# linyicheng1/trackingBench-SLAM

Measured on AMD Instinct MI355X. Metric: frames/sec end-to-end (extract+match+local-BA), higher is better.
Workload: dtype u8 (pyramid/FAST/ORB/Hamming) + f64 (pose-opt/BA); 1 GPU; 1280x720 stereo, 8-level pyramid x0.8, 2000 kpts/image (FAST 80/30), searchByBF L<->R, pose-opt, 10-KF/5000-pt local BA x10 iters; distinct_synthetic_pairs=64, distinct_ba_windows=32, ba_partitions=3, ba_schedule=joined at the end of every step, parallelism=frames sharded x1, RCCL gather of tracks

## Files before the change

### trackingbench_slam_amd/csrc/k_ba.hip

```cpp
#include <mutex>
#include <type_traits>
#include "tb_internal.h"
#include "tb_device.h"
#include "tb_se3.h"

#define BA_T 256
#ifndef BA_KFCH
#define BA_KFCH 512
#endif
#ifndef BA_KFBLK
#define BA_KFBLK 4
#endif
#define BA_BIG_MAXF 64
#define BA_SMALL_MAXF 10
#define BA_SORT_LDS 8192
#ifndef BA_EMAX
#define BA_EMAX 64
#endif
#ifndef BA_PCAP
#define BA_PCAP 21
#endif

struct BaState {
    double lambda, ni, currentChi, chi0, scale_p, rho;
    int iter, qmax, status, need_lin, cur, ok2, done_iters, err;
    int sing, pad0, hq_fresh, pad2;
};

struct BaDims {
    int W, nkf, nfixed, nfree, np, npt, obs_pitch, iters;
    int nblkP, kfChunks, G, nChunks;
    int Gbase, Gextra;
    int Vbase, Vextra;
    int big, npairs;
    unsigned long long oBigA;
    unsigned long long oPairStart, oPairCnt, oPairItems, maxItems;
    double fx, fy, cx, cy;
    unsigned long long wstride, oT, oP, oHll, oBl, oHq, oHpp, oBp, oXp, oPartKF, oPartP, oPartS;
    unsigned long long istride, oPtStart, oPtFree, oKfStart, oKfEdges, oFreeKP;
    unsigned long long oKfRec;
    unsigned long long oPtMask, oPermA, oPermB, oPtRank, oKPs, oGDesc;
    unsigned long long oGCost;
    unsigned long long oGCut;
    int renum;
    unsigned long long oPerm;
    int schurWaveLds;
    int wgReduce;
};

__host__ __device__ inline int ba_schur_waves(const BaDims& d, int w) {
    return d.wgReduce ? 4 * (d.Gbase + (w < d.Gextra ? 1 : 0)) : d.Vbase + (w < d.Vextra ? 1 : 0);
}
__device__ __forceinline__ void ba_schur_unit(int u, int base, int extra, int& w, int& i) {
// ... 2 lines not shown
    else { const int r = u - head; w = extra + r / base; i = r - (w - extra) * base; }
}

typedef double ba_d4 __attribute__((ext_vector_type(4)));
typedef double ba_d2 __attribute__((ext_vector_type(2)));

__device__ __forceinline__ double ba_huber_rho0(double c, double delta) {
    const double dsqr = delta * delta;
    return (c <= dsqr) ? c : 2 * sqrt(c) * delta - dsqr;
}
struct BaLin { double ww, e0, e1, c2, invz; double pc[3]; double Jl[6]; };
__device__ __forceinline__ double ba_rcp(double x) {
    double r = __builtin_amdgcn_rcp(x);
    r = fma(fma(-x, r, 1.0), r, r);
    r = fma(fma(-x, r, 1.0), r, r);
    return r;
}
__device__ __forceinline__ void ba_residual(const double* Rt, const double* X, float u, float v, float inv_sigma2, double fx,
                                            double fy, double cx, double cy, double delta, BaLin& L) {
#pragma unroll
    for (int i = 0; i < 3; i++) L.pc[i] = fma(Rt[3 * i + 2], X[2], fma(Rt[3 * i + 1], X[1], fma(Rt[3 * i], X[0], Rt[9 + i])));
    L.invz = ba_rcp(L.pc[2]);
    L.e0 = (double)u - fma(L.pc[0] * L.invz, fx, cx);
    L.e1 = (double)v - fma(L.pc[1] * L.invz, fy, cy);
    const double wgt = (double)inv_sigma2;
    L.c2 = fma(L.e0, wgt * L.e0, L.e1 * (wgt * L.e1));
    const double r1 = (L.c2 <= delta * delta) ? 1.0 : delta / sqrt(L.c2);
    L.ww = r1 * wgt;
}
__device__ __forceinline__ void ba_linearize(const double* Rt, const double* X, float u, float v, float inv_sigma2, double fx,
// ... 151 lines not shown
            [&](int e, int ce, bool hit) {
                const int prev = (e > 0) ? obs[e - 1].pt : -1, cur = obs[e].pt;
                for (int p = max(prev + 1, 0); p <= min(cur, d.npt); p++) I[d.oPtFree + p] = ce;
                if (hit) {
                    const tb_ba_obs o = obs[e];
                    int4 r;
                    r.x = (int)(((unsigned)cur << 6) | ((unsigned)(o.kf - d.nfixed) & 63u));
                    r.y = __float_as_int(o.u); r.z = __float_as_int(o.v); r.w = __float_as_int(o.inv_sigma2);
                    *reinterpret_cast<int4*>(I + d.oFreeKP + 4 * (size_t)ce) = r;
                }
            });
        for (int p = max((nobs > 0 ? obs[nobs - 1].pt : -1) + 1, 0) + tid; p <= d.npt; p += BA_T) I[d.oPtFree + p] = nfreeE;
        return;
    }
    if (tid == 0) {
        st->lambda = 0; st->ni = 2; st->currentChi = 0; st->chi0 = 0; st->scale_p = 0; st->rho = 0;
        st->iter = 0; st->qmax = 0; st->status = (d.iters > 0 && nobs > 0) ? 0 : 1; st->need_lin = 1; st->cur = 0; st->ok2 = 1;
        st->done_iters = 0; st->err = 0; st->sing = 0; st->hq_fresh = 0;
    }
    __syncthreads();
    if (!d.renum) {
        for (int e = tid; e < nobs; e += BA_T) {
            const int prev = (e > 0) ? obs[e - 1].pt : -1, cur = obs[e].pt;
            for (int p = max(prev + 1, 0); p <= min(cur, d.npt); p++) I[d.oPtStart + p] = e;
        }
        for (int p = max((nobs > 0 ? obs[nobs - 1].pt : -1) + 1, 0) + tid; p <= d.npt; p += BA_T) I[d.oPtStart + p] = nobs;
        if (d.big) for (int p = tid; p < d.npt; p += BA_T) I[d.oPtRank + p] = p;
    }
    for (int kk = tid; kk < d.nkf; kk += BA_T) {
        const float* T = poses + ((size_t)w * d.nkf + kk) * 16;
        double R[9], t[3];
        for (int i = 0; i < 3; i++) { for (int j = 0; j < 3; j++) R[i * 3 + j] = (double)T[i * 4 + j]; t[i] = (double)T[i * 4 + 3]; }
        const PoSE3 s = po_from_Rt(R, t);
        ba_store_se3(D + d.oT + (size_t)kk * 7, s);
        ba_store_se3(D + d.oT + (size_t)(d.nkf + kk) * 7, s);
    }
    for (int i = tid; i < d.npt * 3; i += BA_T) {
        const int r = i / 3, c = i - 3 * r;
        const double v = (double)pts[(size_t)w * d.npt * 3 + (d.renum ? 3 * (size_t)I[d.oPerm + r] + c : (size_t)i)];
        D[d.oP + i] = v;
        D[d.oP + (size_t)d.npt * 3 + i] = v;
    }
}

__device__ __forceinline__ void ba_write_rec(double* q, const double* Hll, const double* bl, const double* X, double lambda,
                                             BaState* st) {
    const double a00 = Hll[0] + lambda, a10 = Hll[1], a20 = Hll[2], a11 = Hll[3] + lambda, a21 = Hll[4], a22 = Hll[5] + lambda;
    bool ok = a00 > 0;
    const double i00 = 1.0 / sqrt(ok ? a00 : 1.0), c10 = a10 * i00, c20 = a20 * i00;
    const double d1 = a11 - c10 * c10;
    ok = ok && d1 > 0;
    const double i11 = 1.0 / sqrt(ok ? d1 : 1.0), c21 = (a21 - c20 * c10) * i11;
    const double d2 = a22 - c20 * c20 - c21 * c21;
    ok = ok && d2 > 0 && isfinite(d2);
    const double i22 = 1.0 / sqrt(ok ? d2 : 1.0);
    if (!ok) st->sing = 1;
    const double u00 = i00, u11 = i11, u22 = i22, u01 = -c10 * i00 * i11, u12 = -c21 * i11 * i22,
                 u02 = -(c20 * i00 + c21 * u01) * i22;
    q[0] = ok ? u00 : 0.0; q[1] = ok ? u01 : 0.0; q[2] = ok ? u02 : 0.0;
    q[3] = ok ? u11 : 0.0; q[4] = ok ? u12 : 0.0; q[5] = ok ? u22 : 0.0;
    q[6] = bl[0]; q[7] = bl[1]; q[8] = bl[2];
    q[9] = X[0]; q[10] = X[1]; q[11] = X[2];
}
__device__ __forceinline__ void ba_rec_utb(const double* q, double* t) {
    t[0] = q[0] * q[6];
    t[1] = q[1] * q[6] + q[3] * q[7];
    t[2] = q[2] * q[6] + q[4] * q[7] + q[5] * q[8];
}

__device__ __forceinline__ void ba_points_pass(const BaDims& d, const tb_ba_obs* __restrict__ obsAll, double* __restrict__ dw, const int* __restrict__ iw,
                                               BaState* __restrict__ states, const int* __restrict__ errflag, int bx, int w) {
    __shared__ double red[4];
    extern __shared__ __attribute__((aligned(16))) double sRt[];
    const int tid = threadIdx.x;
    if (errflag[w]) {
        if (bx == 0 && tid == 0) { states[w].status = 1; states[w].err = 1; }
        return;
    }
    const BaState st = states[w];
    if (st.status) return;
    double* D = dw + (size_t)w * d.wstride;
    const int* I = iw + (size_t)w * d.istride;
    const bool lam_known = st.iter > 0 || !st.need_lin;
    const tb_ba_obs* obs = obsAll + (size_t)w * d.obs_pitch;
    const double* T = D + d.oT + (size_t)st.cur * d.nkf * 7;
    const double* P = D + d.oP + (size_t)st.cur * d.npt * 3;
    for (int k = tid; k < d.nkf; k += BA_T) ba_pose_to_Rt(T + k * 7, sRt + k * 12);
    __syncthreads();
    const double delta = (double)sqrtf(5.991f);
    const int p = bx * BA_T + tid;
    double chi = 0, maxd = 0;
    if (p < d.npt) {
        double Hll[6] = {0, 0, 0, 0, 0, 0}, bl[3] = {0, 0, 0};
        const double X[3] = {P[3 * p], P[3 * p + 1], P[3 * p + 2]};
        const int eBeg = I[d.oPtStart + p], eEnd = I[d.oPtStart + p + 1];
        tb_ba_obs on = obs[min(eBeg, d.obs_pitch - 1)];
        for (int e = eBeg; e < eEnd; e++) {
            const tb_ba_obs o = on;
            on = obs[min(e + 1, d.obs_pitch - 1)];
            BaLin L;
            ba_linearize(sRt + o.kf * 12, X, o.u, o.v, o.inv_sigma2, d.fx, d.fy, d.cx, d.cy, delta, L);
            const double ww = L.ww, e0 = L.e0, e1 = L.e1;
            const double* Jl = L.Jl;
            chi += ba_huber_rho0(L.c2, delta);
            for (int a = 0; a < 3; a++) bl[a] = fma(-ww, fma(Jl[a], e0, Jl[3 + a] * e1), bl[a]);
            Hll[0] = fma(ww, fma(Jl[0], Jl[0], Jl[3] * Jl[3]), Hll[0]);
            Hll[1] = fma(ww, fma(Jl[0], Jl[1], Jl[3] * Jl[4]), Hll[1]);
            Hll[2] = fma(ww, fma(Jl[0], Jl[2], Jl[3] * Jl[5]), Hll[2]);
            Hll[3] = fma(ww, fma(Jl[1], Jl[1], Jl[4] * Jl[4]), Hll[3]);
            Hll[4] = fma(ww, fma(Jl[1], Jl[2], Jl[4] * Jl[5]), Hll[4]);
            Hll[5] = fma(ww, fma(Jl[2], Jl[2], Jl[5] * Jl[5]), Hll[5]);
        }
        if (!lam_known) {
            for (int a = 0; a < 6; a++) D[d.oHll + (size_t)p * 6 + a] = Hll[a];
            for (int a = 0; a < 3; a++) D[d.oBl + (size_t)p * 3 + a] = bl[a];
        } else ba_write_rec(D + d.oHq + (size_t)I[d.oPtRank + p] * 12, Hll, bl, X, st.lambda, states + w);
        maxd = fmax(fabs(Hll[0]), fmax(fabs(Hll[3]), fabs(Hll[5])));
    }
    const double s = ba_block_sum1(chi, red);
    const double m = ba_block_max1(maxd, red);
    if (tid == 0) {
        D[d.oPartP + (size_t)bx * 4] = s;
        D[d.oPartP + (size_t)bx * 4 + 1] = m;
    }
}

#define BA_KFG 14
#define BA_KFR_LDS (4 * (BA_KFG * 65 + 64) + 4 * 27)
__device__ __forceinline__ double ba_block_sum27(const double (&v)[27], double* sh) {
    const int tid = threadIdx.x, wave = tid >> 6, lane = tid & 63;
    double* T = sh + wave * (BA_KFG * 65 + 64);
// ... 75 lines not shown
            for (int a = 0; a < 6; a++) {
                const double wa = ww * Jp[a], wb = ww * Jp[6 + a];
                acc[21 + a] -= fma(wa, e0, wb * e1);
#pragma unroll
                for (int c = a; c < 6; c++) {
                    const int at = a * 6 - (a * (a - 1)) / 2 + (c - a);
                    acc[at] += fma(wa, Jp[c], wb * Jp[6 + c]);
                }
            }
        }
        const double tot = ba_block_sum27(acc, red);
        if (tid < 27) D[d.oPartKF + ((size_t)kfree * d.kfChunks + chunk) * 27 + tid] = tot;
    }
}

__global__ void __launch_bounds__(BA_T)
k_ba_points(BaDims d, const tb_ba_obs* __restrict__ obsAll, double* __restrict__ dw, const int* __restrict__ iw, BaState* __restrict__ states,
            const int* __restrict__ errflag) {
    ba_points_pass(d, obsAll, dw, iw, states, errflag, (int)blockIdx.x, (int)blockIdx.y);
}
__global__ void __launch_bounds__(BA_T)
k_ba_kf(BaDims d, const tb_ba_obs* __restrict__ obsAll, double* __restrict__ dw, const int* __restrict__ iw, const BaState* __restrict__ states,
        const int* __restrict__ errflag) {
    ba_kf_pass(d, obsAll, dw, iw, states, errflag, (int)blockIdx.x);
}
__global__ void __launch_bounds__(BA_T)
k_ba_lin(BaDims d, const tb_ba_obs* __restrict__ obsAll, double* __restrict__ dw, const int* __restrict__ iw, BaState* __restrict__ states,
         const int* __restrict__ errflag, int nKfBlocks) {
    if ((int)blockIdx.x < nKfBlocks) ba_kf_pass(d, obsAll, dw, iw, states, errflag, (int)blockIdx.x);
    else {
        const int b = (int)blockIdx.x - nKfBlocks;
        ba_points_pass(d, obsAll, dw, iw, states, errflag, b % d.nblkP, b / d.nblkP);
    }
}

__device__ __forceinline__ void ba_reduce_body(const BaDims& d, double* __restrict__ dw, const int* __restrict__ iw, BaState* __restrict__ states,
                                               int w, double* red) {
    const int tid = threadIdx.x;
    BaState* st = states + w;
    double* D = dw + (size_t)w * d.wstride;
    const int* I = iw + (size_t)w * d.istride;
    double maxd = 0;
    for (int i = tid; i < d.nfree * 27; i += BA_T) {
        const int kf = i / 27, c = i - kf * 27;
        const int nedges = I[d.oKfStart + d.nfixed + kf + 1] - I[d.oKfStart + d.nfixed + kf];
        const int nch = (nedges + BA_KFCH - 1) / BA_KFCH;
        double s = 0;
        for (int ch = 0; ch < nch; ch++) s += D[d.oPartKF + ((size_t)kf * d.kfChunks + ch) * 27 + c];
        if (c >= 21) D[d.oBp + kf * 6 + (c - 21)] = s;
        else {
            int a = 0, rem = c;
            while (rem >= 6 - a) { rem -= 6 - a; a++; }
            const int b = a + rem;
            D[d.oHpp + (size_t)kf * 36 + a * 6 + b] = s;
            D[d.oHpp + (size_t)kf * 36 + b * 6 + a] = s;
            if (a == b) maxd = fmax(maxd, fabs(s));
        }
    }
    const double mH = ba_block_max1(maxd, red);
    if (tid == 0) {
        double chi = 0, mL = 0;
        for (int b = 0; b < d.nblkP; b++) { chi += D[d.oPartP + (size_t)b * 4]; mL = fmax(mL, D[d.oPartP + (size_t)b * 4 + 1]); }
        st->currentChi = chi;
        if (st->iter == 0) { st->chi0 = chi; st->lambda = 1e-5 * fmax(mH, mL); st->ni = 2; }
        st->hq_fresh = st->iter > 0 ? 1 : 0;
        st->need_lin = 0;
    }
}

__global__ void __launch_bounds__(BA_T)
k_ba_reduce(BaDims d, double* __restrict__ dw, const int* __restrict__ iw, BaState* __restrict__ states) {
    __shared__ double red[4];
    const int w = blockIdx.x;
    if (states[w].status || !states[w].need_lin) return;
    ba_reduce_body(d, dw, iw, states, w, red);
}

__global__ void __launch_bounds__(BA_T)
k_ba_hinv(BaDims d, double* __restrict__ dw, const int* __restrict__ iw, BaState* __restrict__ states) {
    const int w = blockIdx.y, p = blockIdx.x * BA_T + threadIdx.x;
    const BaState st = states[w];
    if (st.status || st.hq_fresh || p >= d.npt) return;
    double* D = dw + (size_t)w * d.wstride;
    const int* I = iw + (size_t)w * d.istride;
    double ph[6], pb[3], X[3];
#pragma unroll
    for (int i = 0; i < 6; i++) ph[i] = D[d.oHll + (size_t)p * 6 + i];
#pragma unroll
    for (int i = 0; i < 3; i++) { pb[i] = D[d.oBl + (size_t)p * 3 + i]; X[i] = D[d.oP + ((size_t)st.cur * d.npt + p) * 3 + i]; }
    ba_write_rec(D + d.oHq + (size_t)I[d.oPtRank + p] * 12, ph, pb, X, st.lambda, states + w);
}

#define BA_MAXT 4
#define BA_REC 12
#define BA_RECS_LDS 256
#define BA_KMFMA 5
#define BA_ZERO_LDS 40
__device__ __forceinline__ void ba_wave_lds_fence() { __builtin_amdgcn_fence(__ATOMIC_SEQ_CST, "wavefront"); }

__host__ __device__ constexpr int ba_c_cap(int k) { return (BA_EMAX / k) < BA_PCAP ? (BA_EMAX / k) : BA_PCAP; }
__host__ __device__ constexpr int ba_c_nb(int k) { return (6 * k + 1 + 3) / 4; }
__host__ __device__ constexpr int ba_c_ld(int k) { return ((3 * ba_c_cap(k) + 3) / 4) * 4 + 2; }
__host__ __device__ constexpr int ba_c_tile(int k) { return 4 * ba_c_nb(k) * ba_c_ld(k); }
#define BA_CB 37
__host__ __device__ constexpr int ba_c_rhs(int k) { return BA_CB * (k * (k + 1) / 2); }
__host__ __device__ constexpr int ba_c_tri(int k) { return ba_c_rhs(k) + 6 * k; }
__host__ __device__ constexpr int ba_c_nacc(int k) {
    const int nb = ba_c_nb(k), nvf = nb / 4, rem = nb % 4;
    return 3 * nvf + 2 * nvf * (nvf - 1) + rem * (nvf + 1);
// ... 613 lines not shown
    const int zeroOfs = d.schurWaveLds - BA_ZERO_LDS;
    double* D = dw + (size_t)w * d.wstride;
    const int* I = iw + (size_t)w * d.istride;
    for (int k = lane; k < d.nfree; k += 64) ba_pose_to_Rt(D + d.oT + ((size_t)st.cur * d.nkf + d.nfixed + k) * 7, sRtf + k * 12);
    double S[36];
#pragma unroll
    for (int e = 0; e < 36; e++) S[e] = 0;
    double rhs = 0;
    int pa = 0;
    while ((pa + 1) * (pa + 2) / 2 <= lane) pa++;
    const int pb = lane - pa * (pa + 1) / 2;
    if (lane < BA_ZERO_LDS) Zt[zeroOfs + lane] = 0;
    ba_wave_lds_fence();
    const double delta = (double)sqrtf(5.991f);
    const int lastE = d.obs_pitch - 1;
    const double* Hq = D + d.oHq;
    const int4* KPs = reinterpret_cast<const int4*>(I + d.oKPs);
    const int4* GD = reinterpret_cast<const int4*>(I + d.oGDesc);
    const unsigned lastQ = (unsigned)d.npt * BA_REC - 1u;
    const int gBeg = I[d.oGCut + wv], gEnd = I[d.oGCut + wv + 1], lastG = gEnd - 1;
    auto range = [&](BaPreC& X, int g) {
        X.nxt = GD[min(g, max(lastG, 0))];
        if (g > lastG) X.nxt.w = 0;
    };
    auto preload = [&](BaPreC& X, int g) {
        const int4 gd = X.nxt;
        const int4 r = KPs[(unsigned)min(gd.y + lane, lastE)];
        X.key = (lane < gd.w * __popc(gd.z)) ? r.x : -1;
        X.u = __int_as_float(r.y); X.v = __int_as_float(r.z); X.w = __int_as_float(r.w);
        const unsigned qb = (unsigned)gd.x * BA_REC + (unsigned)lane;
        X.r0 = Hq[min(qb, lastQ)];
// ... 41 lines not shown
        BA_TK(5);
        const int mask = __builtin_amdgcn_readfirstlane(X.cur.z), npts = __builtin_amdgcn_readfirstlane(X.cur.w);
        const int k = __popc(mask), ld = ba_ctab.ld[k];
        if (pend != 0 && pend != mask) { finish(pend); pend = 0; }
        BA_TK(3);
        Hi[lane] = X.r0;
        Hi[64 + lane] = X.r1;
        Hi[128 + lane] = X.r2;
        Hi[192 + lane] = X.r3;
        ba_wave_lds_fence();
        const bool live = X.key >= 0;
        const int pl = live ? (lane * ((65536 + k - 1) / k)) >> 16 : 0;
        const int slot = live ? lane - pl * k : 0, kf = live ? (X.key & 63) : 0;
        if (live) {
            const double* q = Hi + pl * BA_REC;
            const double u00 = q[0], u01 = q[1], u02 = q[2], u11 = q[3], u12 = q[4], u22 = q[5];
            const double Xp[3] = {q[9], q[10], q[11]};
            BaLin L;
            double Jp[12];
            ba_linearize(sRtf + kf * 12, Xp, X.u, X.v, X.w, d.fx, d.fy, d.cx, d.cy, delta, L);
            ba_jac_pose_iz(L.pc, L.invz, d.fx, d.fy, Jp);
            double JU[6];
#pragma unroll
            for (int r = 0; r < 2; r++) {
                JU[3 * r] = L.Jl[3 * r] * u00;
                JU[3 * r + 1] = fma(L.Jl[3 * r], u01, L.Jl[3 * r + 1] * u11);
                JU[3 * r + 2] = fma(L.Jl[3 * r], u02, fma(L.Jl[3 * r + 1], u12, L.Jl[3 * r + 2] * u22));
            }
            double* z = Zt + (6 * slot) * ld + 3 * pl;
#pragma unroll
            for (int i = 0; i < 6; i++) JU[i] *= L.ww;
#pragma unroll
            for (int a = 0; a < 6; a++) {
#pragma unroll
                for (int c = 0; c < 3; c++)
                    z[a * ld + c] = (a == 3) ? Jp[3] * JU[c] : (a == 4) ? Jp[10] * JU[3 + c] : fma(Jp[a], JU[c], Jp[6 + a] * JU[3 + c]);
            }
            if (slot == 0) {
                double* zr = Zt + (6 * k) * ld + 3 * pl;
                ba_rec_utb(q, zr);
            }
        }
        const int ncol = 3 * npts, nks = (ncol + 3) >> 2;
        if (lane <= 6 * k) {
#pragma unroll
            for (int c = 0; c < 3; c++)
                if (ncol + c < 4 * nks) Zt[lane * ld + ncol + c] = 0;
        }
        ba_wave_lds_fence();
        BA_TK(0);
        preload(X, g + 2);
        BA_TK(1);
        if (k <= BA_KMFMA) {
            switch (k) {
                case 1: ba_c_mac<1>(acc, Zt, nks, lane); break;
// ... 79 lines not shown
        }
    } else {
        double* out = D + d.oPartS + (size_t)wv * 64 * 64;
        if (lane < NPAIR) {
#pragma unroll
            for (int e = 0; e < 36; e++) out[(6 * pa + e / 6) * 64 + 6 * pb + e % 6] = S[e];
        }
        if (lane < d.np) out[lane * 64 + d.np] = rhs;
    }
#ifdef BA_TIMING
    BA_TK(9);
    if (tid == 0 && (w & 15) == 0) { for (int i = 0; i < 10; i++) atomicAdd(&ba_times[i], tk_[i]); atomicAdd(&ba_times[10], 1ull); }
#endif
}

__device__ __forceinline__ double ba_rsqrt(double x) {
    double r = __builtin_amdgcn_rsq(x);
    const double h = 0.5 * x;
    r = fma(r, fma(-h * r, r, 0.5), r);
    r = fma(r, fma(-h * r, r, 0.5), r);
    return r;
}
#define BA_SOLVE_T 256
template <int NS>
__global__ void __launch_bounds__(BA_SOLVE_T)
k_ba_solve(BaDims d, double* __restrict__ dw, const int* __restrict__ iw, BaState* __restrict__ states, int with_reduce) {
    __shared__ double A[64 * 65];
    __shared__ double x[64];
    __shared__ double Lcol[2][64];
    const int w = blockIdx.x, tid = threadIdx.x;
#ifdef BA_TIMING
    unsigned long long ts_[6]; ts_[0] = __builtin_readcyclecounter();
#endif
    BaState* st = states + w;
    if (with_reduce) {
        __shared__ double redf[4];
        if (st->status) return;
// ... 495 lines not shown
    }
    __syncthreads();
    const double* T = D + d.oT + (size_t)st->cur * d.nkf * 7;
    double* Tn = D + d.oT + (size_t)(st->cur ^ 1) * d.nkf * 7;
    for (int k = tid; k < d.nkf; k += BA_ST) {
        const PoSE3 Tk = ba_load_se3(T + k * 7);
        if (k < d.nfixed) ba_store_se3(Tn + k * 7, Tk);
        else {
            double u[6];
            for (int a = 0; a < 6; a++) u[a] = xs[6 * (k - d.nfixed) + a];
            ba_store_se3(Tn + k * 7, po_exp_mul(u, Tk));
        }
    }
}

__global__ void __launch_bounds__(BA_T)
k_ba_update(BaDims d, const tb_ba_obs* __restrict__ obsAll, double* __restrict__ dw, const int* __restrict__ iw,
            const BaState* __restrict__ states) {
    __shared__ double red[4];
    extern __shared__ __attribute__((aligned(16))) double sdyn[];
    double* const sRt = sdyn;
    double* const sRtc = sdyn + (size_t)d.nkf * 12;
    double* const sx = sdyn + (size_t)d.nkf * 24;
    const int w = blockIdx.y, tid = threadIdx.x;
    const BaState st = states[w];
    if (st.status) return;
    const tb_ba_obs* obs = obsAll + (size_t)w * d.obs_pitch;
    double* D = dw + (size_t)w * d.wstride;
    const int* I = iw + (size_t)w * d.istride;
    const double* Tn = D + d.oT + (size_t)(st.cur ^ 1) * d.nkf * 7;
    for (int k = tid; k < d.nkf; k += BA_T) ba_pose_to_Rt(D + d.oT + ((size_t)st.cur * d.nkf + k) * 7, sRtc + k * 12);
    const double* P = D + d.oP + (size_t)st.cur * d.npt * 3;
    double* Pn = D + d.oP + (size_t)(st.cur ^ 1) * d.npt * 3;
    for (int k = tid; k < d.nkf; k += BA_T) ba_pose_to_Rt(Tn + k * 7, sRt + k * 12);
    for (int i = tid; i < d.np; i += BA_T) sx[i] = D[d.oXp + i];
    __syncthreads();
    const double delta = (double)sqrtf(5.991f);
    const int p = blockIdx.x * BA_T + tid;
    double chi = 0, sc = 0;
    if (p < d.npt) {
        const double* q = D + d.oHq + (size_t)I[d.oPtRank + p] * 12;
        double r[3] = {q[6], q[7], q[8]};
        const double bl[3] = {r[0], r[1], r[2]};
        double xl[3] = {0, 0, 0};
        const int eBeg = I[d.oPtStart + p], eEnd = I[d.oPtStart + p + 1];
        if (st.ok2) {
            const double u00 = q[0], u01 = q[1], u02 = q[2], u11 = q[3], u12 = q[4], u22 = q[5];
            const double Xc[3] = {P[3 * p], P[3 * p + 1], P[3 * p + 2]};
            tb_ba_obs on = obs[min(eBeg, d.obs_pitch - 1)];
            for (int e = eBeg; e < eEnd; e++) {
                const tb_ba_obs o = on;
                on = obs[min(e + 1, d.obs_pitch - 1)];
                if (o.kf < d.nfixed) continue;
                BaLin L;
                double Jp[12];
                ba_linearize(sRtc + o.kf * 12, Xc, o.u, o.v, o.inv_sigma2, d.fx, d.fy, d.cx, d.cy, delta, L);
                ba_jac_pose_iz(L.pc, L.invz, d.fx, d.fy, Jp);
                const double* xp = sx + 6 * (o.kf - d.nfixed);
                double s0 = 0, s1 = 0;
#pragma unroll
                for (int a = 0; a < 6; a++) { s0 = fma(Jp[a], xp[a], s0); s1 = fma(Jp[6 + a], xp[a], s1); }
#pragma unroll
                for (int c = 0; c < 3; c++) r[c] = fma(-L.ww, fma(L.Jl[c], s0, L.Jl[3 + c] * s1), r[c]);
            }
            const double t0 = u00 * r[0], t1 = u01 * r[0] + u11 * r[1], t2 = u02 * r[0] + u12 * r[1] + u22 * r[2];
            xl[0] = u00 * t0 + u01 * t1 + u02 * t2;
            xl[1] = u11 * t1 + u12 * t2;
            xl[2] = u22 * t2;
        }
        double X[3];
        for (int a = 0; a < 3; a++) {
            X[a] = P[3 * p + a] + xl[a];
            Pn[3 * p + a] = X[a];
            sc += xl[a] * (st.lambda * xl[a] + bl[a]);
        }
        tb_ba_obs on2 = obs[min(eBeg, d.obs_pitch - 1)];
        for (int e = eBeg; e < eEnd; e++) {
            const tb_ba_obs o = on2;
            on2 = obs[min(e + 1, d.obs_pitch - 1)];
            BaLin L;
            ba_residual(sRt + o.kf * 12, X, o.u, o.v, o.inv_sigma2, d.fx, d.fy, d.cx, d.cy, delta, L);
            chi += ba_huber_rho0(L.c2, delta);
        }
    }
    const double s1 = ba_block_sum1(chi, red);
    const double s2 = ba_block_sum1(sc, red);
    if (tid == 0) {
        D[d.oPartP + (size_t)blockIdx.x * 4 + 2] = s1;
        D[d.oPartP + (size_t)blockIdx.x * 4 + 3] = s2;
    }
}

__global__ void __launch_bounds__(64)
k_ba_decide(BaDims d, const double* __restrict__ dw, BaState* __restrict__ states, int* __restrict__ running) {
    const int w = blockIdx.x, lane = threadIdx.x;
    BaState* st = states + w;
    if (st->status) return;
    const double* D = dw + (size_t)w * d.wstride;
    double tc = 0, sc = 0;
    for (int b = lane; b < d.nblkP; b += 64) { tc += D[d.oPartP + (size_t)b * 4 + 2]; sc += D[d.oPartP + (size_t)b * 4 + 3]; }
    tc = po_wave_sum(tc);
    sc = po_wave_sum(sc);
    if (lane != 0) return;
    double tempChi = tc, scale = st->scale_p + sc;
    if (!st->ok2) tempChi = 1.7976931348623157e308;
    scale += 1e-3;
    const double rho = (st->currentChi - tempChi) / scale;
    if (rho > 0 && isfinite(tempChi)) {
        double alpha = 1. - pow(2 * rho - 1, 3);
        alpha = fmin(alpha, 2. / 3.);
        st->lambda *= fmax(1. / 3., alpha);
        st->ni = 2;
        st->currentChi = tempChi;
        st->cur ^= 1;
        st->need_lin = 1;
    } else {
        st->lambda *= st->ni;
        st->ni *= 2;
    }
    st->qmax++;
    st->rho = rho;
    st->sing = 0;
    st->hq_fresh = 0;
    if (!(rho < 0 && st->qmax < 10)) {
        st->done_iters++;
        const bool terminate = (st->qmax == 10 || rho == 0);
        st->iter++;
        st->qmax = 0;
        st->need_lin = 1;
        if (terminate || st->iter >= d.iters) st->status = 1;
    }
    if (!st->status) atomicAdd(running, 1);
}

__global__ void __launch_bounds__(BA_T)
k_ba_finish(BaDims d, const double* __restrict__ dw, const int* __restrict__ iw, const BaState* __restrict__ states,
            float* __restrict__ poses, float* __restrict__ pts, double* __restrict__ stats) {
    const int w = blockIdx.x, tid = threadIdx.x;
// ... 42 lines not shown
        d.wgReduce = d.Gbase > 4 ? 1 : 0;
        const int T = 4 * std::max(slots, W);
        d.Vbase = std::min(T / std::max(W, 1), 4 * cap);
        d.Vextra = d.Vbase < 4 * cap ? T % std::max(W, 1) : 0;
    }
    d.big = d.nfree > BA_SMALL_MAXF;
    d.renum = (!d.big && npt <= BA_SORT_LDS && nkf <= BA_PREP_MAXKF) ? 1 : 0;
    d.schurWaveLds = d.big ? 0 : ba_c_wave_lds(d.nfree);
    d.npairs = d.nfree * (d.nfree + 1) / 2;
    d.maxItems = (unsigned long long)obs_pitch * (d.nfree + 1) / 2 + 1;
    d.fx = K[0]; d.fy = K[1]; d.cx = K[2]; d.cy = K[3];
    unsigned long long o = 0;
    auto take = [&](unsigned long long n) { unsigned long long r = o; o += (n + 1) & ~1ull; return r; };
    d.oT = take(2ull * nkf * 7);
    d.oP = take(2ull * npt * 3);
    d.oHll = take(6ull * npt);
    d.oBl = take(3ull * npt);
    d.oHq = take(12ull * npt);
    d.oHpp = take(36ull * std::max(d.nfree, 1));
    d.oBp = take(std::max(64, d.np));
    d.oXp = take(std::max(64, d.np));
    d.oPartKF = take(27ull * std::max(d.nfree, 1) * d.kfChunks);
    d.oPartP = take(4ull * d.nblkP);
    const int maxWaves = d.wgReduce ? 4 * d.G : d.Vbase + (d.Vextra > 0 ? 1 : 0);
    d.oPartS = take(d.big ? 0 : 4096ull * (d.wgReduce ? d.G : maxWaves));
    d.oBigA = take(d.big ? (unsigned long long)(d.np + 1) * d.np + 32 : 0);
    d.wstride = o;
    unsigned long long io = 0;
    auto itake = [&](unsigned long long n) { unsigned long long r = io; io += (n + 3) & ~3ull; return r; };
    d.oPtStart = itake(npt + 1);
    d.oPtFree = itake(npt + 1);
    d.oKfStart = itake(nkf + 1);
    d.oKfEdges = itake(obs_pitch);
// ... 69 lines not shown
        if (d.renum) {
        } else if (!d.big) {
            tb_prof_begin(ctx, "k_ba_groups");
            hipLaunchKernelGGL(k_ba_groups, dim3(W), dim3(BA_T), 0, s, d, iw, errflag);
            tb_prof_end(ctx);
        } else {
            tb_prof_begin(ctx, "k_ba_pairs");
            hipLaunchKernelGGL(k_ba_pairs<false>, dim3(d.nfree, W), dim3(64), 0, s, d, d_obs, iw, errflag);
            hipLaunchKernelGGL(k_ba_pair_scan, dim3(W), dim3(BA_T), 0, s, d, iw, errflag);
            hipLaunchKernelGGL(k_ba_pairs<true>, dim3(d.nfree, W), dim3(64), 0, s, d, d_obs, iw, errflag);
            tb_prof_end(ctx);
        }
        TB_HIP(ctx, hipGetLastError());
        return TB_OK;
    };
    auto enqueue_round = [&](int round) -> int {
        {
            const int nKfBlocks = ((W + 7) / 8) * 8 * std::min(BA_KFBLK, d.kfChunks) * d.nfree;
            if (W <= 32) {
                tb_prof_begin(ctx, "k_ba_lin");
                hipLaunchKernelGGL(k_ba_lin, dim3(nKfBlocks + d.nblkP * W), dim3(BA_T), (size_t)d.nkf * 12 * sizeof(double), s, d, d_obs, dw, iw, states,
                                   errflag, nKfBlocks);
                tb_prof_end(ctx);
            } else {
                tb_prof_begin(ctx, "k_ba_points");
                hipLaunchKernelGGL(k_ba_points, dim3(d.nblkP, W), dim3(BA_T), (size_t)d.nkf * 12 * sizeof(double), s, d, d_obs, dw, iw, states, errflag);
                tb_prof_end(ctx);
                tb_prof_begin(ctx, "k_ba_kf");
                hipLaunchKernelGGL(k_ba_kf, dim3(nKfBlocks), dim3(BA_T), 0, s, d, d_obs, dw, iw, states, errflag);
                tb_prof_end(ctx);
            }
        }
        const bool reduce_in_solve = !d.big && round > 0;
        if (!reduce_in_solve) {
            tb_prof_begin(ctx, "k_ba_reduce");
            hipLaunchKernelGGL(k_ba_reduce, dim3(W), dim3(BA_T), 0, s, d, dw, iw, states);
            tb_prof_end(ctx);
        }
        if (round == 0) {
            tb_prof_begin(ctx, "k_ba_hinv");
            hipLaunchKernelGGL(k_ba_hinv, dim3(d.nblkP, W), dim3(BA_T), 0, s, d, dw, iw, states);
            tb_prof_end(ctx);
        }
        if (d.big) {
            tb_prof_begin(ctx, "k_ba_schur_pairs");
            hipLaunchKernelGGL(k_ba_schur_pairs, dim3((d.npairs + 3) / 4, W), dim3(BA_T), 0, s, d, dw, iw, states);
            tb_prof_end(ctx);
            tb_prof_begin(ctx, "k_ba_solve_big");
            hipLaunchKernelGGL(k_ba_solve_big, dim3(W), dim3(BA_ST), big_lds, s, d, dw, states);
            tb_prof_end(ctx);
        } else {
            tb_prof_begin(ctx, "k_ba_schur");
            hipLaunchKernelGGL(ks, dim3(d.wgReduce ? d.Gbase * W + d.Gextra : (d.Vbase * W + d.Vextra + 3) / 4), dim3(BA_T), schur_lds, s, d, dw, iw, states);
            tb_prof_end(ctx);
            tb_prof_begin(ctx, "k_ba_solve");
            if (d.np <= 16) hipLaunchKernelGGL(k_ba_solve<16>, dim3(W), dim3(BA_SOLVE_T), 0, s, d, dw, iw, states, reduce_in_solve ? 1 : 0);
            else if (d.np <= 32) hipLaunchKernelGGL(k_ba_solve<32>, dim3(W), dim3(BA_SOLVE_T), 0, s, d, dw, iw, states, reduce_in_solve ? 1 : 0);
            else if (d.np <= 48) hipLaunchKernelGGL(k_ba_solve<48>, dim3(W), dim3(BA_SOLVE_T), 0, s, d, dw, iw, states, reduce_in_solve ? 1 : 0);
            else hipLaunchKernelGGL(k_ba_solve<64>, dim3(W), dim3(BA_SOLVE_T), 0, s, d, dw, iw, states, reduce_in_solve ? 1 : 0);
            tb_prof_end(ctx);
        }
        tb_prof_begin(ctx, "k_ba_update");
        hipLaunchKernelGGL(k_ba_update, dim3(d.nblkP, W), dim3(BA_T), ((size_t)d.nkf * 24 + d.np) * sizeof(double), s, d, d_obs, dw, iw, states);
        tb_prof_end(ctx);
        tb_prof_begin(ctx, "k_ba_decide");
        hipLaunchKernelGGL(k_ba_decide, dim3(W), dim3(64), 0, s, d, dw, states, running + round % ring);
        tb_prof_end(ctx);
        TB_HIP(ctx, hipGetLastError());
        return TB_OK;
    };
    int host_running = 1, rounds = 0, rc = TB_OK;
    const int max_rounds = std::min(iters * 10 + 1, 1000);
    int batch = iters;
    const bool use_graph = W <= 32 && !ctx->prof && std::min(batch, max_rounds) > 0;
    if (use_graph) {
        struct Key { BaDims d; const void *poses, *pts, *obs, *counts, *work; hipStream_t s; } key;
        memset(&key, 0, sizeof key);
        key.d = d; key.poses = d_poses; key.pts = d_pts; key.obs = d_obs_in; key.counts = d_counts; key.work = d_work; key.s = s;
// ... 44 lines not shown
```

Before: 30670 frames/s.

## Fuse point relinearization into BA update and drop separate point pass

For the small-BA path, the update kernel now relinearizes each point at its trial position and writes raw Hll/bl/X records into a double-buffered slot, so the next round skips the separate point linearization pass. The per-point Cholesky is recomputed on the fly from the raw record, in the Schur and update kernels, using the current lambda. This removes the hinv kernel and the separate Hll/Bl arrays. The trade-off is recomputing the 3x3 factor per use, a fast rsqrt approximation, and wasted relinearization work whenever a step is rejected.

```diff
diff --git a/trackingbench_slam_amd/csrc/k_ba.hip b/trackingbench_slam_amd/csrc/k_ba.hip
--- a/trackingbench_slam_amd/csrc/k_ba.hip
+++ b/trackingbench_slam_amd/csrc/k_ba.hip
@@ -13,6 +13,7 @@
 #endif
 #define BA_BIG_MAXF 64
 #define BA_SMALL_MAXF 10
+#define BA_REC 12
 #define BA_SORT_LDS 8192
 #ifndef BA_EMAX
 #define BA_EMAX 64
@@ -23,8 +24,9 @@
 
 struct BaState {
     double lambda, ni, currentChi, chi0, scale_p, rho;
+    double chiNext;
     int iter, qmax, status, need_lin, cur, ok2, done_iters, err;
-    int sing, pad0, hq_fresh, pad2;
+    int sing, pad0, pad1, pad2;
 };
 
 struct BaDims {
@@ -36,7 +38,7 @@
     unsigned long long oBigA;
     unsigned long long oPairStart, oPairCnt, oPairItems, maxItems;
     double fx, fy, cx, cy;
-    unsigned long long wstride, oT, oP, oHll, oBl, oHq, oHpp, oBp, oXp, oPartKF, oPartP, oPartS;
+    unsigned long long wstride, oT, oP, oHq, oHpp, oBp, oXp, oPartKF, oPartP, oPartS;
     unsigned long long istride, oPtStart, oPtFree, oKfStart, oKfEdges, oFreeKP;
     unsigned long long oKfRec;
     unsigned long long oPtMask, oPermA, oPermB, oPtRank, oKPs, oGDesc;
@@ -69,6 +71,13 @@
     double r = __builtin_amdgcn_rcp(x);
     r = fma(fma(-x, r, 1.0), r, r);
     r = fma(fma(-x, r, 1.0), r, r);
+    return r;
+}
+__device__ __forceinline__ double ba_rsqrt(double x) {
+    double r = __builtin_amdgcn_rsq(x);
+    const double h = 0.5 * x;
+    r = fma(r, fma(-h * r, r, 0.5), r);
+    r = fma(r, fma(-h * r, r, 0.5), r);
     return r;
 }
 __device__ __forceinline__ void ba_residual(const double* Rt, const double* X, float u, float v, float inv_sigma2, double fx,
@@ -250,9 +259,9 @@
         return;
     }
     if (tid == 0) {
-        st->lambda = 0; st->ni = 2; st->currentChi = 0; st->chi0 = 0; st->scale_p = 0; st->rho = 0;
+        st->lambda = 0; st->ni = 2; st->currentChi = 0; st->chi0 = 0; st->scale_p = 0; st->rho = 0; st->chiNext = 0;
         st->iter = 0; st->qmax = 0; st->status = (d.iters > 0 && nobs > 0) ? 0 : 1; st->need_lin = 1; st->cur = 0; st->ok2 = 1;
-        st->done_iters = 0; st->err = 0; st->sing = 0; st->hq_fresh = 0;
+        st->done_iters = 0; st->err = 0; st->sing = 0;
     }
     __syncthreads();
     if (!d.renum) {
@@ -279,24 +288,67 @@
     }
 }
 
+#ifndef BA_REC_EXACT
+#define BA_REC_EXACT 0
+#endif
+__device__ __forceinline__ double ba_rec_isqrt(double x) {
+#if BA_REC_EXACT
+    return 1.0 / sqrt(x);
+#else
+    return ba_rsqrt(x);
+#endif
+}
+__device__ __forceinline__ void ba_rec_u(const double* Hll, double lambda, double* U, bool& ok) {
+    const double a00 = Hll[0] + lambda, a10 = Hll[1], a20 = Hll[2], a11 = Hll[3] + lambda, a21 = Hll[4], a22 = Hll[5] + lambda;
+    ok = a00 > 0;
+    const double i00 = ba_rec_isqrt(ok ? a00 : 1.0), c10 = a10 * i00, c20 = a20 * i00;
+    const double d1 = a11 - c10 * c10;
+    ok = ok && d1 > 0;
+    const double i11 = ba_rec_isqrt(ok ? d1 : 1.0), c21 = (a21 - c20 * c10) * i11;
+    const double d2 = a22 - c20 * c20 - c21 * c21;
+    ok = ok && d2 > 0 && isfinite(d2);
+    const double i22 = ba_rec_isqrt(ok ? d2 : 1.0);
+    const double u00 = i00, u11 = i11, u22 = i22, u01 = -c10 * i00 * i11, u12 = -c21 * i11 * i22,
+                 u02 = -(c20 * i00 + c21 * u01) * i22;
+    U[0] = ok ? u00 : 0.0; U[1] = ok ? u01 : 0.0; U[2] = ok ? u02 : 0.0;
+    U[3] = ok ? u11 : 0.0; U[4] = ok ? u12 : 0.0; U[5] = ok ? u22 : 0.0;
+}
 __device__ __forceinline__ void ba_write_rec(double* q, const double* Hll, const double* bl, const double* X, double lambda,
                                              BaState* st) {
-    const double a00 = Hll[0] + lambda, a10 = Hll[1], a20 = Hll[2], a11 = Hll[3] + lambda, a21 = Hll[4], a22 = Hll[5] + lambda;
-    bool ok = a00 > 0;
-    const double i00 = 1.0 / sqrt(ok ? a00 : 1.0), c10 = a10 * i00, c20 = a20 * i00;
-    const double d1 = a11 - c10 * c10;
-    ok = ok && d1 > 0;
-    const double i11 = 1.0 / sqrt(ok ? d1 : 1.0), c21 = (a21 - c20 * c10) * i11;
-    const double d2 = a22 - c20 * c20 - c21 * c21;
-    ok = ok && d2 > 0 && isfinite(d2);
-    const double i22 = 1.0 / sqrt(ok ? d2 : 1.0);
+    double U[6];
+    bool ok;
+    ba_rec_u(Hll, lambda, U, ok);
     if (!ok) st->sing = 1;
-    const double u00 = i00, u11 = i11, u22 = i22, u01 = -c10 * i00 * i11, u12 = -c21 * i11 * i22,
-                 u02 = -(c20 * i00 + c21 * u01) * i22;
-    q[0] = ok ? u00 : 0.0; q[1] = ok ? u01 : 0.0; q[2] = ok ? u02 : 0.0;
-    q[3] = ok ? u11 : 0.0; q[4] = ok ? u12 : 0.0; q[5] = ok ? u22 : 0.0;
+#pragma unroll
+    for (int a = 0; a < 6; a++) q[a] = U[a];
     q[6] = bl[0]; q[7] = bl[1]; q[8] = bl[2];
     q[9] = X[0]; q[10] = X[1]; q[11] = X[2];
+}
+__device__ __forceinline__ void ba_point_edge(const BaDims& d, const double* Rt, const double* X, const tb_ba_obs& o, double delta,
+                                              double* Hll, double* bl, double& chi) {
+    BaLin L;
+    ba_linearize(Rt, X, o.u, o.v, o.inv_sigma2, d.fx, d.fy, d.cx, d.cy, delta, L);
+    const double ww = L.ww, e0 = L.e0, e1 = L.e1;
+    const double* Jl = L.Jl;
+    chi += ba_huber_rho0(L.c2, delta);
+#pragma unroll
+    for (int a = 0; a < 3; a++) bl[a] = fma(-ww, fma(Jl[a], e0, Jl[3 + a] * e1), bl[a]);
+    Hll[0] = fma(ww, fma(Jl[0], Jl[0], Jl[3] * Jl[3]), Hll[0]);
+    Hll[1] = fma(ww, fma(Jl[0], Jl[1], Jl[3] * Jl[4]), Hll[1]);
+    Hll[2] = fma(ww, fma(Jl[0], Jl[2], Jl[3] * Jl[5]), Hll[2]);
+    Hll[3] = fma(ww, fma(Jl[1], Jl[1], Jl[4] * Jl[4]), Hll[3]);
+    Hll[4] = fma(ww, fma(Jl[1], Jl[2], Jl[4] * Jl[5]), Hll[4]);
+    Hll[5] = fma(ww, fma(Jl[2], Jl[2], Jl[5] * Jl[5]), Hll[5]);
+}
+__device__ __forceinline__ void ba_write_rec_lin(double* q, const double* Hll, const double* bl, const double* X) {
+    ba_d2* q2 = reinterpret_cast<ba_d2*>(q);
+    q2[0] = ba_d2{Hll[0], Hll[1]}; q2[1] = ba_d2{Hll[2], Hll[3]}; q2[2] = ba_d2{Hll[4], Hll[5]};
+    q2[3] = ba_d2{bl[0], bl[1]}; q2[4] = ba_d2{bl[2], X[0]}; q2[5] = ba_d2{X[1], X[2]};
+}
+__device__ __forceinline__ void ba_u_utb(const double* U, const double* bl, double* t) {
+    t[0] = U[0] * bl[0];
+    t[1] = U[1] * bl[0] + U[3] * bl[1];
+    t[2] = U[2] * bl[0] + U[4] * bl[1] + U[5] * bl[2];
 }
 __device__ __forceinline__ void ba_rec_utb(const double* q, double* t) {
     t[0] = q[0] * q[6];
@@ -304,6 +356,7 @@
     t[2] = q[2] * q[6] + q[4] * q[7] + q[5] * q[8];
 }
 
+template <bool LF>
 __device__ __forceinline__ void ba_points_pass(const BaDims& d, const tb_ba_obs* __restrict__ obsAll, double* __restrict__ dw, const int* __restrict__ iw,
                                                BaState* __restrict__ states, const int* __restrict__ errflag, int bx, int w) {
     __shared__ double red[4];
@@ -334,23 +387,11 @@
         for (int e = eBeg; e < eEnd; e++) {
             const tb_ba_obs o = on;
             on = obs[min(e + 1, d.obs_pitch - 1)];
-            BaLin L;
-            ba_linearize(sRt + o.kf * 12, X, o.u, o.v, o.inv_sigma2, d.fx, d.fy, d.cx, d.cy, delta, L);
-            const double ww = L.ww, e0 = L.e0, e1 = L.e1;
-            const double* Jl = L.Jl;
-            chi += ba_huber_rho0(L.c2, delta);
-            for (int a = 0; a < 3; a++) bl[a] = fma(-ww, fma(Jl[a], e0, Jl[3 + a] * e1), bl[a]);
-            Hll[0] = fma(ww, fma(Jl[0], Jl[0], Jl[3] * Jl[3]), Hll[0]);
-            Hll[1] = fma(ww, fma(Jl[0], Jl[1], Jl[3] * Jl[4]), Hll[1]);
-            Hll[2] = fma(ww, fma(Jl[0], Jl[2], Jl[3] * Jl[5]), Hll[2]);
-            Hll[3] = fma(ww, fma(Jl[1], Jl[1], Jl[4] * Jl[4]), Hll[3]);
-            Hll[4] = fma(ww, fma(Jl[1], Jl[2], Jl[4] * Jl[5]), Hll[4]);
-            Hll[5] = fma(ww, fma(Jl[2], Jl[2], Jl[5] * Jl[5]), Hll[5]);
-        }
-        if (!lam_known) {
-            for (int a = 0; a < 6; a++) D[d.oHll + (size_t)p * 6 + a] = Hll[a];
-            for (int a = 0; a < 3; a++) D[d.oBl + (size_t)p * 3 + a] = bl[a];
-        } else ba_write_rec(D + d.oHq + (size_t)I[d.oPtRank + p] * 12, Hll, bl, X, st.lambda, states + w);
+            ba_point_edge(d, sRt + o.kf * 12, X, o, delta, Hll, bl, chi);
+        }
+        double* q = D + d.oHq + (size_t)I[d.oPtRank + p] * BA_REC;
+        if constexpr (LF) ba_write_rec_lin(q + (size_t)st.cur * d.npt * BA_REC, Hll, bl, X);
+        else if (lam_known) ba_write_rec(q, Hll, bl, X, st.lambda, states + w);
         maxd = fmax(fabs(Hll[0]), fmax(fabs(Hll[3]), fabs(Hll[5])));
     }
     const double s = ba_block_sum1(chi, red);
@@ -456,23 +497,25 @@
     }
 }
 
+template <bool LF>
 __global__ void __launch_bounds__(BA_T)
 k_ba_points(BaDims d, const tb_ba_obs* __restrict__ obsAll, double* __restrict__ dw, const int* __restrict__ iw, BaState* __restrict__ states,
             const int* __restrict__ errflag) {
-    ba_points_pass(d, obsAll, dw, iw, states, errflag, (int)blockIdx.x, (int)blockIdx.y);
+    ba_points_pass<LF>(d, obsAll, dw, iw, states, errflag, (int)blockIdx.x, (int)blockIdx.y);
 }
 __global__ void __launch_bounds__(BA_T)
 k_ba_kf(BaDims d, const tb_ba_obs* __restrict__ obsAll, double* __restrict__ dw, const int* __restrict__ iw, const BaState* __restrict__ states,
         const int* __restrict__ errflag) {
     ba_kf_pass(d, obsAll, dw, iw, states, errflag, (int)blockIdx.x);
 }
+template <bool LF>
 __global__ void __launch_bounds__(BA_T)
 k_ba_lin(BaDims d, const tb_ba_obs* __restrict__ obsAll, double* __restrict__ dw, const int* __restrict__ iw, BaState* __restrict__ states,
          const int* __restrict__ errflag, int nKfBlocks) {
     if ((int)blockIdx.x < nKfBlocks) ba_kf_pass(d, obsAll, dw, iw, states, errflag, (int)blockIdx.x);
     else {
         const int b = (int)blockIdx.x - nKfBlocks;
-        ba_points_pass(d, obsAll, dw, iw, states, errflag, b % d.nblkP, b / d.nblkP);
+        ba_points_pass<LF>(d, obsAll, dw, iw, states, errflag, b % d.nblkP, b / d.nblkP);
     }
 }
 
@@ -503,9 +546,9 @@
     if (tid == 0) {
         double chi = 0, mL = 0;
         for (int b = 0; b < d.nblkP; b++) { chi += D[d.oPartP + (size_t)b * 4]; mL = fmax(mL, D[d.oPartP + (size_t)b * 4 + 1]); }
-        st->currentChi = chi;
+        if (d.big || st->iter == 0) st->chiNext = chi;
+        st->currentChi = st->chiNext;
         if (st->iter == 0) { st->chi0 = chi; st->lambda = 1e-5 * fmax(mH, mL); st->ni = 2; }
-        st->hq_fresh = st->iter > 0 ? 1 : 0;
         st->need_lin = 0;
     }
 }
@@ -518,23 +561,7 @@
     ba_reduce_body(d, dw, iw, states, w, red);
 }
 
-__global__ void __launch_bounds__(BA_T)
-k_ba_hinv(BaDims d, double* __restrict__ dw, const int* __restrict__ iw, BaState* __restrict__ states) {
-    const int w = blockIdx.y, p = blockIdx.x * BA_T + threadIdx.x;
-    const BaState st = states[w];
-    if (st.status || st.hq_fresh || p >= d.npt) return;
-    double* D = dw + (size_t)w * d.wstride;
-    const int* I = iw + (size_t)w * d.istride;
-    double ph[6], pb[3], X[3];
-#pragma unroll
-    for (int i = 0; i < 6; i++) ph[i] = D[d.oHll + (size_t)p * 6 + i];
-#pragma unroll
-    for (int i = 0; i < 3; i++) { pb[i] = D[d.oBl + (size_t)p * 3 + i]; X[i] = D[d.oP + ((size_t)st.cur * d.npt + p) * 3 + i]; }
-    ba_write_rec(D + d.oHq + (size_t)I[d.oPtRank + p] * 12, ph, pb, X, st.lambda, states + w);
-}
-
 #define BA_MAXT 4
-#define BA_REC 12
 #define BA_RECS_LDS 256
 #define BA_KMFMA 5
 #define BA_ZERO_LDS 40
@@ -1178,7 +1205,7 @@
     ba_wave_lds_fence();
     const double delta = (double)sqrtf(5.991f);
     const int lastE = d.obs_pitch - 1;
-    const double* Hq = D + d.oHq;
+    const double* Hq = D + d.oHq + (size_t)st.cur * d.npt * BA_REC;
     const int4* KPs = reinterpret_cast<const int4*>(I + d.oKPs);
     const int4* GD = reinterpret_cast<const int4*>(I + d.oGDesc);
     const unsigned lastQ = (unsigned)d.npt * BA_REC - 1u;
@@ -1250,7 +1277,11 @@
         const int slot = live ? lane - pl * k : 0, kf = live ? (X.key & 63) : 0;
         if (live) {
             const double* q = Hi + pl * BA_REC;
-            const double u00 = q[0], u01 = q[1], u02 = q[2], u11 = q[3], u12 = q[4], u22 = q[5];
+            double U[6];
+            bool ok;
+            ba_rec_u(q, st.lambda, U, ok);
+            if (!ok) states[w].sing = 1;
+            const double u00 = U[0], u01 = U[1], u02 = U[2], u11 = U[3], u12 = U[4], u22 = U[5];
             const double Xp[3] = {q[9], q[10], q[11]};
             BaLin L;
             double Jp[12];
@@ -1274,7 +1305,7 @@
             }
             if (slot == 0) {
                 double* zr = Zt + (6 * k) * ld + 3 * pl;
-                ba_rec_utb(q, zr);
+                ba_u_utb(U, q + 6, zr);
             }
         }
         const int ncol = 3 * npts, nks = (ncol + 3) >> 2;
@@ -1384,13 +1415,6 @@
 #endif
 }
 
-__device__ __forceinline__ double ba_rsqrt(double x) {
-    double r = __builtin_amdgcn_rsq(x);
-    const double h = 0.5 * x;
-    r = fma(r, fma(-h * r, r, 0.5), r);
-    r = fma(r, fma(-h * r, r, 0.5), r);
-    return r;
-}
 #define BA_SOLVE_T 256
 template <int NS>
 __global__ void __launch_bounds__(BA_SOLVE_T)
@@ -1916,9 +1940,10 @@
     }
 }
 
+template <bool LF>
 __global__ void __launch_bounds__(BA_T)
 k_ba_update(BaDims d, const tb_ba_obs* __restrict__ obsAll, double* __restrict__ dw, const int* __restrict__ iw,
-            const BaState* __restrict__ states) {
+            BaState* __restrict__ states) {
     __shared__ double red[4];
     extern __shared__ __attribute__((aligned(16))) double sdyn[];
     double* const sRt = sdyn;
@@ -1941,14 +1966,34 @@
     const int p = blockIdx.x * BA_T + tid;
     double chi = 0, sc = 0;
     if (p < d.npt) {
-        const double* q = D + d.oHq + (size_t)I[d.oPtRank + p] * 12;
+        const size_t slot = (size_t)I[d.oPtRank + p] * BA_REC;
+        const double* qg = D + d.oHq + (LF ? (size_t)st.cur * d.npt * BA_REC : (size_t)0) + slot;
+        double q[BA_REC];
+        if constexpr (LF) {
+            const ba_d2* q2 = reinterpret_cast<const ba_d2*>(qg);
+#pragma unroll
+            for (int a = 0; a < BA_REC / 2; a++) { const ba_d2 v = q2[a]; q[2 * a] = v.x; q[2 * a + 1] = v.y; }
+        } else {
+#pragma unroll
+            for (int a = 0; a < BA_REC; a++) q[a] = qg[a];
+        }
         double r[3] = {q[6], q[7], q[8]};
         const double bl[3] = {r[0], r[1], r[2]};
         double xl[3] = {0, 0, 0};
+        const double Xc[3] = {LF ? q[9] : P[3 * p], LF ? q[10] : P[3 * p + 1], LF ? q[11] : P[3 * p + 2]};
         const int eBeg = I[d.oPtStart + p], eEnd = I[d.oPtStart + p + 1];
         if (st.ok2) {
-            const double u00 = q[0], u01 = q[1], u02 = q[2], u11 = q[3], u12 = q[4], u22 = q[5];
-            const double Xc[3] = {P[3 * p], P[3 * p + 1], P[3 * p + 2]};
+            double U[6];
+            if constexpr (LF) {
+                const double Hc[6] = {q[0], q[1], q[2], q[3], q[4], q[5]};
+                bool ok;
+                ba_rec_u(Hc, st.lambda, U, ok);
+                if (!ok) states[w].sing = 1;
+            } else {
+#pragma unroll
+                for (int a = 0; a < 6; a++) U[a] = q[a];
+            }
+            const double u00 = U[0], u01 = U[1], u02 = U[2], u11 = U[3], u12 = U[4], u22 = U[5];
             tb_ba_obs on = obs[min(eBeg, d.obs_pitch - 1)];
             for (int e = eBeg; e < eEnd; e++) {
                 const tb_ba_obs o = on;
@@ -1972,17 +2017,27 @@
         }
         double X[3];
         for (int a = 0; a < 3; a++) {
-            X[a] = P[3 * p + a] + xl[a];
+            X[a] = Xc[a] + xl[a];
             Pn[3 * p + a] = X[a];
             sc += xl[a] * (st.lambda * xl[a] + bl[a]);
         }
         tb_ba_obs on2 = obs[min(eBeg, d.obs_pitch - 1)];
-        for (int e = eBeg; e < eEnd; e++) {
-            const tb_ba_obs o = on2;
-            on2 = obs[min(e + 1, d.obs_pitch - 1)];
-            BaLin L;
-            ba_residual(sRt + o.kf * 12, X, o.u, o.v, o.inv_sigma2, d.fx, d.fy, d.cx, d.cy, delta, L);
-            chi += ba_huber_rho0(L.c2, delta);
+        if constexpr (LF) {
+            double Hn[6] = {0, 0, 0, 0, 0, 0}, bn[3] = {0, 0, 0};
+            for (int e = eBeg; e < eEnd; e++) {
+                const tb_ba_obs o = on2;
+                on2 = obs[min(e + 1, d.obs_pitch - 1)];
+                ba_point_edge(d, sRt + o.kf * 12, X, o, delta, Hn, bn, chi);
+            }
+            ba_write_rec_lin(D + d.oHq + (size_t)(st.cur ^ 1) * d.npt * BA_REC + slot, Hn, bn, X);
+        } else {
+            for (int e = eBeg; e < eEnd; e++) {
+                const tb_ba_obs o = on2;
+                on2 = obs[min(e + 1, d.obs_pitch - 1)];
+                BaLin L;
+                ba_residual(sRt + o.kf * 12, X, o.u, o.v, o.inv_sigma2, d.fx, d.fy, d.cx, d.cy, delta, L);
+                chi += ba_huber_rho0(L.c2, delta);
+            }
         }
     }
     const double s1 = ba_block_sum1(chi, red);
@@ -1999,13 +2054,19 @@
     BaState* st = states + w;
     if (st->status) return;
     const double* D = dw + (size_t)w * d.wstride;
-    double tc = 0, sc = 0;
-    for (int b = lane; b < d.nblkP; b += 64) { tc += D[d.oPartP + (size_t)b * 4 + 2]; sc += D[d.oPartP + (size_t)b * 4 + 3]; }
+    double tc = 0, sc = 0, chiNext = 0;
+    for (int b0 = 0; b0 < d.nblkP; b0 += 64) {
+        const int b = b0 + lane;
+        const double c = b < d.nblkP ? D[d.oPartP + (size_t)b * 4 + 2] : 0.0;
+        tc += c;
+        if (b < d.nblkP) sc += D[d.oPartP + (size_t)b * 4 + 3];
+        for (int j = 0; j < min(64, d.nblkP - b0); j++) chiNext += __shfl(c, j, 64);
+    }
     tc = po_wave_sum(tc);
     sc = po_wave_sum(sc);
     if (lane != 0) return;
     double tempChi = tc, scale = st->scale_p + sc;
-    if (!st->ok2) tempChi = 1.7976931348623157e308;
+    if (!st->ok2 || st->sing) { tempChi = 1.7976931348623157e308; scale = 0; }
     scale += 1e-3;
     const double rho = (st->currentChi - tempChi) / scale;
     if (rho > 0 && isfinite(tempChi)) {
@@ -2014,6 +2075,7 @@
         st->lambda *= fmax(1. / 3., alpha);
         st->ni = 2;
         st->currentChi = tempChi;
+        st->chiNext = chiNext;
         st->cur ^= 1;
         st->need_lin = 1;
     } else {
@@ -2023,7 +2085,6 @@
     st->qmax++;
     st->rho = rho;
     st->sing = 0;
-    st->hq_fresh = 0;
     if (!(rho < 0 && st->qmax < 10)) {
         st->done_iters++;
         const bool terminate = (st->qmax == 10 || rho == 0);
@@ -2096,9 +2157,7 @@
     auto take = [&](unsigned long long n) { unsigned long long r = o; o += (n + 1) & ~1ull; return r; };
     d.oT = take(2ull * nkf * 7);
     d.oP = take(2ull * npt * 3);
-    d.oHll = take(6ull * npt);
-    d.oBl = take(3ull * npt);
-    d.oHq = take(12ull * npt);
+    d.oHq = take((d.big ? 1ull : 2ull) * BA_REC * npt);
     d.oHpp = take(36ull * std::max(d.nfree, 1));
     d.oBp = take(std::max(64, d.np));
     d.oXp = take(std::max(64, d.np));
@@ -2198,18 +2257,25 @@
         TB_HIP(ctx, hipGetLastError());
         return TB_OK;
     };
+    typedef void (*points_t)(BaDims, const tb_ba_obs*, double*, const int*, BaState*, const int*);
+    const points_t kp = d.big ? (points_t)k_ba_points<false> : (points_t)k_ba_points<true>;
     auto enqueue_round = [&](int round) -> int {
         {
             const int nKfBlocks = ((W + 7) / 8) * 8 * std::min(BA_KFBLK, d.kfChunks) * d.nfree;
-            if (W <= 32) {
+            const bool points = d.big || round == 0;
+            if (points && W <= 32) {
                 tb_prof_begin(ctx, "k_ba_lin");
-                hipLaunchKernelGGL(k_ba_lin, dim3(nKfBlocks + d.nblkP * W), dim3(BA_T), (size_t)d.nkf * 12 * sizeof(double), s, d, d_obs, dw, iw, states,
-                                   errflag, nKfBlocks);
+                if (d.big) hipLaunchKernelGGL(k_ba_lin<false>, dim3(nKfBlocks + d.nblkP * W), dim3(BA_T), (size_t)d.nkf * 12 * sizeof(double), s, d, d_obs, dw, iw, states,
+                                              errflag, nKfBlocks);
+                else hipLaunchKernelGGL(k_ba_lin<true>, dim3(nKfBlocks + d.nblkP * W), dim3(BA_T), (size_t)d.nkf * 12 * sizeof(double), s, d, d_obs, dw, iw, states,
+                                        errflag, nKfBlocks);
                 tb_prof_end(ctx);
             } else {
-                tb_prof_begin(ctx, "k_ba_points");
-                hipLaunchKernelGGL(k_ba_points, dim3(d.nblkP, W), dim3(BA_T), (size_t)d.nkf * 12 * sizeof(double), s, d, d_obs, dw, iw, states, errflag);
-                tb_prof_end(ctx);
+                if (points) {
+                    tb_prof_begin(ctx, "k_ba_points");
+                    hipLaunchKernelGGL(kp, dim3(d.nblkP, W), dim3(BA_T), (size_t)d.nkf * 12 * sizeof(double), s, d, d_obs, dw, iw, states, errflag);
+                    tb_prof_end(ctx);
+                }
                 tb_prof_begin(ctx, "k_ba_kf");
                 hipLaunchKernelGGL(k_ba_kf, dim3(nKfBlocks), dim3(BA_T), 0, s, d, d_obs, dw, iw, states, errflag);
                 tb_prof_end(ctx);
@@ -2221,9 +2287,9 @@
             hipLaunchKernelGGL(k_ba_reduce, dim3(W), dim3(BA_T), 0, s, d, dw, iw, states);
             tb_prof_end(ctx);
         }
-        if (round == 0) {
-            tb_prof_begin(ctx, "k_ba_hinv");
-            hipLaunchKernelGGL(k_ba_hinv, dim3(d.nblkP, W), dim3(BA_T), 0, s, d, dw, iw, states);
+        if (d.big && round == 0) {
+            tb_prof_begin(ctx, "k_ba_points");
+            hipLaunchKernelGGL(kp, dim3(d.nblkP, W), dim3(BA_T), (size_t)d.nkf * 12 * sizeof(double), s, d, d_obs, dw, iw, states, errflag);
             tb_prof_end(ctx);
         }
         if (d.big) {
@@ -2245,7 +2311,8 @@
             tb_prof_end(ctx);
         }
         tb_prof_begin(ctx, "k_ba_update");
-        hipLaunchKernelGGL(k_ba_update, dim3(d.nblkP, W), dim3(BA_T), ((size_t)d.nkf * 24 + d.np) * sizeof(double), s, d, d_obs, dw, iw, states);
+        if (d.big) hipLaunchKernelGGL(k_ba_update<false>, dim3(d.nblkP, W), dim3(BA_T), ((size_t)d.nkf * 24 + d.np) * sizeof(double), s, d, d_obs, dw, iw, states);
+        else hipLaunchKernelGGL(k_ba_update<true>, dim3(d.nblkP, W), dim3(BA_T), ((size_t)d.nkf * 24 + d.np) * sizeof(double), s, d, d_obs, dw, iw, states);
         tb_prof_end(ctx);
         tb_prof_begin(ctx, "k_ba_decide");
         hipLaunchKernelGGL(k_ba_decide, dim3(W), dim3(64), 0, s, d, dw, states, running + round % ring);
```

Result: no change. 30650 frames/s (-0.0%).
